# JJanai/back2future

Measured on AMD Instinct MI355X. Metric: frame-triplets/sec at 3x1024x1920, higher is better.
Workload: dtype f32; 1 GPU; BASELINE.json configs[4] per-GPU share: batch=16 synthetic 3x1024x1920 triplets per GPU, random-init pwc.lua weights (Ours-Hard shape), outputs flow + occ + est[3]; batch_per_gpu=16, global_batch=16, height=1024, width=1920, parallelism=dp1: independent triplets per rank, one RCCL weight broadcast at init, hip_graph=True

## Files before the change

back2future_amd/csrc/b2f_api.hip:

```cpp
#include "b2f_ctx.h"

#include <cctype>
#include <cmath>
#include <cstdio>
#include <cstdlib>

using namespace b2f;

static thread_local std::string g_err;
namespace b2f {
int api_fail(const std::string &m)
{
    g_err = m;
    return 1;
}
const std::string &api_error() { return g_err; }

ConvSeg cp8_seg(const float *ptr, int C, size_t hw)
{
    ConvSeg sgm;
    sgm.ptr = ptr;
    sgm.img_stride = (long)(hw * (size_t)((C + 7) / 8 * 8));
    sgm.chunk_stride = (long)(hw * 8);
    sgm.pix_stride = 8;
// ... 240 lines not shown
    return 0;
}

int find_conv(const b2f_ctx *c, int kind, int level, int idx)
{
    for (size_t i = 0; i < c->lay.size(); ++i)
        if (c->lay[i].kind == kind && c->lay[i].level == level && c->lay[i].idx == idx) return (int)i;
    return -1;
}

struct Plan {
    int B, H, W;
    bool full;
    bool seq;
    bool stream;
    bool past;
    int nimg;
    int fo;
    int rec;
    int h[8], w[8];
    size_t img, tmp, cs[8], U[8], UB[8], cv, d[6], fs, bfs, logits, u2, flow_planar, ds[6], total;
};

Plan make_plan(int B, int H, int W, bool full, bool past_flow, bool seq = false, bool stream = false, bool want_past = false)
{
    Plan p;
    p.B = B; p.H = H; p.W = W;
    p.full = full;
    p.seq = seq;
    p.stream = stream;
    p.past = past_flow && (full || want_past);
    p.nimg = stream ? B : seq ? B + 2 : 3 * B;
    p.fo = seq ? 1 : B;
    p.rec = kCvRec;
    for (int l = 1; l <= 7; ++l) { p.h[l] = H >> (l - 1); p.w[l] = W >> (l - 1); }
    size_t off = 0;
    auto take = [&](size_t n) { size_t o = off; off += (n + 63) & ~(size_t)63; return o; };
    p.img = full ? take((size_t)3 * B * H * W * kImgC) : 0;
    p.tmp = take((size_t)p.nimg * p.h[2] * p.w[2] * kFeat[2]);
    for (int l = 2; l <= 7; ++l) p.cs[l] = take((stream && l >= 3) ? 0 : (size_t)p.nimg * p.h[l] * p.w[l] * kFeat[l]);
    for (int l = 3; l <= 6; ++l) p.U[l] = take((size_t)B * p.h[l] * p.w[l] * 2);
    for (int l = 3; l <= 6; ++l) p.UB[l] = p.past ? take((size_t)B * p.h[l] * p.w[l] * 2) : 0;
    p.cv = take((size_t)B * p.h[3] * p.w[3] * p.rec + 64);
    const size_t px3 = (size_t)B * p.h[3] * p.w[3];
    for (int i = 1; i <= 5; ++i) p.d[i] = take(px3 * kDec[i]);
    p.fs = take(px3 * 8);
    p.bfs = take(px3 * 8);
    p.logits = take(px3 * 8);
    p.u2 = take(px3 * 4 * 2);
    p.flow_planar = take((size_t)B * 2 * H * W);
    for (int k = 2; k <= 5; ++k) p.ds[k] = full ? take((size_t)2 * B * (H >> (k - 1)) * (W >> (k - 1)) * kImgC) : 0;
    p.total = off;
    return p;
}

}
void b2f::drop_gen_out(b2f_ctx *c)
{
    for (float *p : c->gen_out)
        if (p) (void)hipFree(p);
    c->gen_out.clear();
    c->genB = c->genH = c->genW = 0;
}
void b2f::drop_graphs(b2f_ctx *c)
// ... 120 lines not shown
{
    const PackedConv &p = c->packed[conv_id];
    ConvLaunch L{};
    for (int i = 0; i < p.nseg; ++i) L.seg[i] = segs[i];
    L.out = out;
    L.H = H; L.W = W; L.stride = stride;
    const size_t hwo = (size_t)((H + 2 - 3) / stride + 1) * ((W + 2 - 3) / stride + 1);
    L.out_img_stride = (long)(hwo * ((p.cout + 7) / 8 * 8));
    L.out_chunk_stride = (long)(hwo * 8);
    L.out_pix_stride = 8;
    L.nimg = nimg;
    L.leaky = leaky;
    return launch_layer(c, s, !cap, p, c->wpk_dev, *c, c->cur_batch, L);
}

int run_decoder(b2f_ctx *c, hipStream_t s, bool cap, const Plan &P, const float *ref, int kind, int l, float *out2)
{
    const size_t *dbuf = P.d;
    float *A = c->arena;
    const int h = P.h[l], w = P.w[l], B = P.B;
    const size_t hw = (size_t)h * w;
    const int Cl = kFeat[l];
    const int id1 = find_conv(c, kind, l, 1);
    if (id1 < 0) return fail("decoder not present in this model");
    ConvSeg segs[2];
    const ConvSeg seg_ref = cp8_seg(ref, Cl, hw);
    const ConvSeg seg_cv = cp8_seg(A + P.cv, kCvRec, hw);
    if (c->packed[id1].nseg == 2) { segs[0] = seg_ref; segs[1] = seg_cv; }
    else { segs[0] = seg_cv; segs[1] = seg_cv; }
    CHK(run_conv(c, s, cap, id1, segs, B, h, w, 1, 1, A + dbuf[1]));
    for (int i = 2; i <= 6; ++i) {
        const ConvSeg in = cp8_seg(A + dbuf[i - 1], kDec[i - 1], hw);
        float *o = (i == 6) ? out2 : A + dbuf[i];
        CHK(run_conv(c, s, cap, find_conv(c, kind, l, i), &in, B, h, w, 1, i < 6, o));
    }
    return 0;
}

struct Feat {
    float *pyr[8];
    const float *past[8], *ref[8], *fut[8];
};

Feat make_feat(const b2f_ctx *c, const Plan &P, const StreamPass *sp)
{
    Feat F{};
    for (int l = 2; l <= 7; ++l) {
        const size_t img = (size_t)P.h[l] * P.w[l] * kFeat[l];
        if (sp && l >= 3) {
            F.pyr[l] = sp->pyr[l];
            F.past[l] = sp->past[l]; F.ref[l] = sp->ref[l]; F.fut[l] = sp->fut[l];
// ... 7 lines not shown

struct Outs {
    float *flow = nullptr, *occ = nullptr, *est3 = nullptr;
    float *past = nullptr;
    float *t_ufs[8] = {nullptr}, *t_ubfs[8] = {nullptr}, *t_occ[8] = {nullptr}, *t_iw1[8] = {nullptr}, *t_iw3[8] = {nullptr};
};

int forward_impl(b2f_ctx *c, hipStream_t s, bool cap, const void *dev_in, int in_kind, const Plan &P, const Outs &O, const StreamPass *sp = nullptr)
{
    c->cur_batch = c->req_batch > 0 ? c->req_batch : P.B;
    float *A = c->arena;
    const Feat F = make_feat(c, P, sp);
    const int B = P.B;
    const bool full = P.full, past = P.past;
    const int unit = in_kind == B2F_IN_UNIT;
    if (full) {
        Scope sc(c, s, "pack_input", cap);
        HIPCHK(launch_pack_input((const float *)dev_in, unit, B, P.H, P.W, A + P.img, s));
    }
    const int head_id1 = find_conv(c, KIND_FEAT, 2, 2), head_id2 = find_conv(c, KIND_FEAT, 3, 1);
    const bool head_fused = c->bf16_direct >= 2 && P.h[2] >= 4 && P.w[2] >= 4 && head_id1 >= 0 && head_id2 >= 0 &&
                            c->packed[(size_t)head_id1].base == K_C16 && c->packed[(size_t)head_id2].base == K_C16S2;
    for (int l = 2; l <= 7; ++l) {
        const int hi = P.h[l - 1], wi = P.w[l - 1], ho = P.h[l], wo = P.w[l];
        const int Ci = (l == 2) ? kImgC : kFeat[l - 1], Co = kFeat[l];
        if (l == 2 && (P.seq || sp)) {
            Scope sc(c, s, "conv_first_seq", cap);
            HIPCHK(launch_conv_first_seq(dev_in, in_kind, P.nimg, P.H, P.W, c->wpk_dev + c->first_w_off, c->wpk_dev + c->first_b_off,
                                         A + P.tmp, s));
        } else if (l == 2) {
// ... 56 lines not shown
        cl.out = A + P.cv;
        cl.out_img_stride = (long)(hw * kCvRec);
        cl.out_chunk_stride = (long)(hw * 8);
        cl.out_pix_stride = 8;
        cl.B = B; cl.C = Cl; cl.h = h; cl.w = w;
        cl.variant = c->corr_variant;
        cl.ablate = c->corr_ablate;
        {
            char cname[48];
            snprintf(cname, sizeof cname, c->profile_layers ? "warp_costvol_%dx%d" : "warp_costvol", h, w);
            Scope sc(c, s, cname, cap);
            HIPCHK(launch_warp_costvol(cl, s));
        }
        float *occ_out = full ? O.t_occ[l] : (l == 3 ? O.occ : nullptr);
        float *occ_out2 = (!full && l == 3 && c->past_flow) ? O.est3 : nullptr;
        if (occ_out || occ_out2) {
            CHK(run_decoder(c, s, cap, P, F.ref[l], KIND_OCC, l, A + P.logits));
            {
                Scope sc(c, s, "softmax_nearest4", cap);
                if (occ_out) HIPCHK(launch_softmax_nearest4_planar(A + P.logits, 8, B, h, w, occ_out, s));
                if (occ_out2) HIPCHK(launch_softmax_nearest4_planar(A + P.logits, 8, B, h, w, occ_out2, s));
            }
        }
        CHK(run_decoder(c, s, cap, P, F.ref[l], KIND_FLOW, l, A + P.fs));
        if (past) CHK(run_decoder(c, s, cap, P, F.ref[l], KIND_PAST, l, A + P.bfs));
        float *skip_f = full ? O.t_ufs[l] : (l == 3 ? (O.flow ? O.flow : A + P.flow_planar) : nullptr);
        {
            Scope sc(c, s, "upsample_flow2x", cap);
            float *u = (l > 3) ? A + P.U[l - 1] : A + P.u2;
            HIPCHK(launch_upsample_flow2x(A + P.fs, 8, B, h, w, u, s));
            if (skip_f) HIPCHK(launch_upsample_flow2x_planar(u, 2, B, 2 * h, 2 * w, skip_f, s));
            if (past) {
                float *ub = (l > 3) ? A + P.UB[l - 1] : A + P.d[1];
                HIPCHK(launch_upsample_flow2x(A + P.bfs, 8, B, h, w, ub, s));
                float *skip_b = full ? O.t_ubfs[l] : (l == 3 ? O.past : nullptr);
                if (skip_b) HIPCHK(launch_upsample_flow2x_planar(ub, 2, B, 2 * h, 2 * w, skip_b, s));
            }
// ... 3 lines not shown
            const int k = l - 2;
            const int hk = 4 * h, wk = 4 * w;
            const size_t img_f = (size_t)B * hk * wk * kImgC;
            const float *im1 = (k == 1) ? A + P.img : A + P.ds[k];
            const float *im3 = (k == 1) ? A + P.img + 2 * img_f : A + P.ds[k] + img_f;
            const float kk = (float)(20.0 / std::pow(2.0, l - 3));
            const float *fl1 = (past && O.t_ubfs[l]) ? O.t_ubfs[l] : O.t_ufs[l];
            if (O.t_iw1[l]) HIPCHK(launch_warp_image_planar(im1, fl1, -kk, B, hk, wk, O.t_iw1[l], s));
            if (O.t_iw3[l]) HIPCHK(launch_warp_image_planar(im3, O.t_ufs[l], kk, B, hk, wk, O.t_iw3[l], s));
        }
    }
    if (!full && O.est3 && !c->past_flow && (P.seq || sp)) {
        Scope sc(c, s, "warp_image_seq", cap);
        HIPCHK(launch_warp_input_seq(sp ? sp->frame_past : dev_in, sp ? sp->frame_kind : in_kind, O.flow ? O.flow : A + P.flow_planar, -20.0f, B,
                                     P.H, P.W, O.est3, s));
    } else if (!full && O.est3 && !c->past_flow) {
        Scope sc(c, s, "warp_image", cap);
        HIPCHK(launch_warp_input_planar((const float *)dev_in, unit, 0, O.flow ? O.flow : A + P.flow_planar, -20.0f, B, P.H, P.W,
                                        O.est3, s));
    }
    return 0;
}

}
int b2f::find_conv_id(const b2f_ctx *c, int kind, int level, int idx) { return find_conv(c, kind, level, idx); }
int b2f::run_conv_layer(b2f_ctx *c, hipStream_t s, bool cap, int conv_id, const ConvSeg *segs, int nimg, int H, int W, int stride,
                        int leaky, float *out)
{
    if (conv_id < 0) return fail("b2f: layer not present in this model");
    return run_conv(c, s, cap, conv_id, segs, nimg, H, W, stride, leaky, out);
}
// ... 76 lines not shown
    {"bf16_conv_min_pixels", &b2f_ctx::bf16_conv_min_pixels, OPT_SYNC, 0},
    {"wino1d", &b2f_ctx::wino1d, OPT_ENV | OPT_SYNC, 2},
    {"wino6", &b2f_ctx::wino6, OPT_ENV | OPT_SYNC, 3},
    {"wino6_min_pixels", &b2f_ctx::wino6_min_pixels, OPT_ENV | OPT_SYNC, 0},
    {"wino2_split", &b2f_ctx::wino2_split, OPT_ENV | OPT_SYNC | OPT_EXP_ONLY, 4},
    {"wino4_split", &b2f_ctx::wino4_split, OPT_ENV | OPT_SYNC | OPT_EXP_ONLY, 5},
    {"wino4_hybrid", &b2f_ctx::wino4_hybrid, OPT_ENV | OPT_SYNC | OPT_EXP_ONLY, 5},
    {"s2_tiles_per_block", &b2f_ctx::s2_tiles_per_block, OPT_ENV | OPT_SYNC, 0},
    {"wino4_persistent", &b2f_ctx::wino4_persistent, OPT_ENV | OPT_SYNC, 0},
    {"s2_loader", &b2f_ctx::s2_loader, OPT_ENV | OPT_SYNC, 0},
    {"s2_tile_groups", &b2f_ctx::s2_tile_groups, OPT_ENV | OPT_SYNC, 0},
    {"wino_split_pixels", &b2f_ctx::wino_split_pixels, OPT_ENV | OPT_SYNC, 0},
    {"wino8", &b2f_ctx::wino8, OPT_ENV | OPT_SYNC, 0},
    {"wino4_min_pixels", &b2f_ctx::wino4_min_pixels, OPT_ENV | OPT_SYNC, 0},
    {"adaptive_kernels", &b2f_ctx::adaptive_kernels, OPT_ENV | OPT_SYNC, 0},
    {"op_wino_split", &b2f_ctx::op_wino_split, OPT_ENV, 0},
    {"op_hole_fill", &b2f_ctx::op_hole_fill, 0, 0},
    {"host_subbatch_pixels", nullptr, OPT_ENV, 0},
    {"host_threads", &b2f_ctx::host_threads, OPT_ENV, 0},
    {"host_u8", &b2f_ctx::host_u8, OPT_ENV, 0},
    {"host_ramp", &b2f_ctx::host_ramp, OPT_ENV, 0},
    {"debug_fail_next", &b2f_ctx::debug_fail_next, 0, 0},
};

const OptRow *find_option(const char *key)
{
    for (const OptRow &r : kOptions)
        if (!strcmp(key, r.name)) return &r;
    return nullptr;
}
// ... 350 lines not shown
                    drop_gen_out(c);
                    return fail("b2f_forward_device: out of device memory");
                }
            }
            c->genB = B; c->genH = H; c->genW = W;
        }
        std::vector<float *> &dev = c->gen_out;
        CHK(graph_forward(c, s, false, dev_in, in_kind, B, H, W, dev.data()));
        const size_t n2 = (size_t)B * 2 * H * W * sizeof(float);
        if (dev_flow) HIPCHK(hipMemcpyAsync(dev_flow, dev[0], n2, hipMemcpyDeviceToDevice, s));
        if (dev_occ) HIPCHK(hipMemcpyAsync(dev_occ, dev[(size_t)(c->past_flow ? 2 : 1)], n2, hipMemcpyDeviceToDevice, s));
        if (dev_est3) HIPCHK(hipMemcpyAsync(dev_est3, dev[2], c->past_flow ? n2 : n2 / 2 * 3, hipMemcpyDeviceToDevice, s));
        if (dev_past) HIPCHK(hipMemcpyAsync(dev_past, dev[1], n2, hipMemcpyDeviceToDevice, s));
        return 0;
    }
    const Plan P = make_plan(B, H, W, false, c->past_flow, seq, sp != nullptr, dev_past != nullptr);
    CHK(ensure_workspace(c, P));
    Outs O;
    O.flow = dev_flow; O.occ = dev_occ; O.est3 = dev_est3; O.past = dev_past;
    if (graph && !c->profile) {
        if (c->graphs.size() > 256) {
            HIPCHK(hipDeviceSynchronize());
            drop_graphs(c);
        }
        const int req = c->req_batch > 0 ? c->req_batch : B;
        const GraphKey key = {dev_in, dev_flow, dev_occ, dev_est3, in_kind, B, H, W, (c->adaptive_kernels > 0 || (c->adaptive_kernels < 0 && req == 1)) ? 1 : 0,
                              seq ? 1 : 0, sp ? sp->ring : nullptr, sp ? 1 + 2 * sp->slot + (sp->ready ? 1 : 0) : 0, dev_past};
        auto it = c->graphs.find(key);
        if (it == c->graphs.end()) {
            c->graphs.emplace(key, nullptr);
            return forward_impl(c, s, false, dev_in, in_kind, P, O, sp);
// ... 664 lines not shown
```

back2future_amd/csrc/b2f_ctx.h:

```cpp
#pragma once
#include "../../include/b2f.h"

#include <algorithm>
#include <atomic>
#include <condition_variable>
#include <cstring>
#include <exception>
#include <map>
#include <memory>
#include <mutex>
#include <string>
#include <thread>
#include <tuple>
#include <vector>

#include "b2f_host.h"
#include "b2f_internal.h"

namespace b2f {

int api_fail(const std::string &m);
const std::string &api_error();


// ... 357 lines not shown
    float *wpk_dev = nullptr;
    size_t wpk_floats = 0;
    size_t first_w_off = 0, first_b_off = 0;
    float *arena = nullptr;
    size_t arena_floats = 0;
    int wsB = 0, wsH = 0, wsW = 0;
    int use_graph = 0, profile = 0;
    int host_graph = 1;
    int cur_batch = 0;
    int req_batch = 0;
    int corr_ablate = 0;
    int corr_variant = -1;
    int op_wino_split = 0;
    int op_hole_fill = 0;
    int profile_layers = 0;
    long long host_subbatch_pixels = 16ll << 20;
    int host_threads = 0;
    int host_u8 = 1, host_ramp = 1;
    int debug_fail_next = 0;
    std::map<b2f::GraphKey, hipGraphExec_t> graphs;
    std::vector<float *> gen_out;
    int genB = 0, genH = 0, genW = 0;
    std::vector<std::string> prof_names;
    std::vector<double> prof_ms;
    std::vector<long long> prof_n;
    std::vector<b2f::ProfEvent> prof_pending;
    std::vector<hipEvent_t> ev_pool;
    hipStream_t s_in = nullptr, s_out = nullptr;
    b2f::HostSlot slot[2];
    std::unique_ptr<b2f::CopyPool> pool_in, pool_out;
// ... 46 lines not shown
```

back2future_amd/csrc/b2f_glue.hip:

```cpp
#include "b2f_internal.h"

namespace b2f {

__global__ void pack_input_kernel(const float *in, int normalize, int B, int H, int W, float *img)
{
    const size_t hw = (size_t)H * W;
    const size_t i = (size_t)blockIdx.x * blockDim.x + threadIdx.x;
    if (i >= (size_t)B * hw) return;
    const size_t b = i / hw, p = i - b * hw;
#pragma unroll
    for (int f = 0; f < 3; ++f) {
        float v[3];
#pragma unroll
        for (int c = 0; c < 3; ++c) {
            float x = in[(b * 9 + f * 3 + c) * hw + p];
            if (normalize) x = color_normalize(x, c);
            v[c] = x;
        }
        float4 *o = reinterpret_cast<float4 *>(img + (((size_t)f * B + b) * hw + p) * kImgC);
        o[0] = make_float4(v[0], v[1], v[2], 0.f);
        o[1] = make_float4(0.f, 0.f, 0.f, 0.f);
    }
}

// ... 30 lines not shown
    const float bl = y1 ? src[(size_t)iw * pix_stride] : 0.f;
    const float br = (x1 && y1) ? src[(size_t)(iw + 1) * pix_stride] : 0.f;
    out[pix * out_pix_stride + c] = wx * wy * tl + (1.f - wx) * wy * tr + wx * (1.f - wy) * bl + (1.f - wx) * (1.f - wy) * br;
}

hipError_t launch_warp_nhwc(const float *img, long img_stride, int pix_stride, int C, int ih, int iw,
                            const float *grid, float k, int B, int gh, int gw, float *out,
                            int out_pix_stride, hipStream_t s)
{
    const size_t n = (size_t)B * gh * gw * C;
    hipLaunchKernelGGL(warp_nhwc_kernel, dim3((unsigned)((n + 255) / 256)), dim3(256), 0, s, img, img_stride,
                       pix_stride, C, ih, iw, grid, k, B, gh, gw, out, out_pix_stride);
    return hipGetLastError();
}

__device__ __forceinline__ float2 bilerp2(const float *in, int ps, int h, int w, float rh, float rw, int y2, int x2)
{
    const float h1r = rh * (float)y2;
    const int h1 = (int)h1r;
    const int h1p = (h1 < h - 1) ? 1 : 0;
    const float h1l = h1r - (float)h1, h0l = 1.f - h1l;
    const float w1r = rw * (float)x2;
    const int w1 = (int)w1r;
    const int w1p = (w1 < w - 1) ? 1 : 0;
    const float w1l = w1r - (float)w1, w0l = 1.f - w1l;
    const float *p = in + ((size_t)h1 * w + w1) * ps;
    const float2 a = *reinterpret_cast<const float2 *>(p), b = *reinterpret_cast<const float2 *>(p + (size_t)w1p * ps);
    const float2 c = *reinterpret_cast<const float2 *>(p + (size_t)h1p * w * ps);
    const float2 d = *reinterpret_cast<const float2 *>(p + ((size_t)h1p * w + w1p) * ps);
    float2 o;
    o.x = h0l * (w0l * a.x + w1l * b.x) + h1l * (w0l * c.x + w1l * d.x);
    o.y = h0l * (w0l * a.y + w1l * b.y) + h1l * (w0l * c.y + w1l * d.y);
    return o;
}

__global__ __launch_bounds__(256) void upsample_flow2x_kernel(const float *in, int ps, int B, int h, int w, float *out, int planar)
{
    const int H2 = 2 * h, W2 = 2 * w;
    const int x0 = 4 * (int)(blockIdx.x * blockDim.x + threadIdx.x);
    const int y2 = (int)blockIdx.y, b = (int)blockIdx.z;
    if (x0 >= W2) return;
    const float rh = (H2 > 1) ? (float)(h - 1) / (float)(H2 - 1) : 0.f;
    const float rw = (W2 > 1) ? (float)(w - 1) / (float)(W2 - 1) : 0.f;
    const float *src = in + (size_t)b * h * w * ps;
    float2 o[4];
#pragma unroll
    for (int k = 0; k < 4; ++k) o[k] = bilerp2(src, ps, h, w, rh, rw, y2, min(x0 + k, W2 - 1));
    const size_t hw2 = (size_t)H2 * W2, row = (size_t)y2 * W2 + x0;
    if (planar) {
        float *o0 = out + ((size_t)b * 2) * hw2 + row, *o1 = o0 + hw2;
        if ((W2 & 3) == 0) {
            *reinterpret_cast<float4 *>(o0) = make_float4(o[0].x, o[1].x, o[2].x, o[3].x);
            *reinterpret_cast<float4 *>(o1) = make_float4(o[0].y, o[1].y, o[2].y, o[3].y);
        } else {
#pragma unroll
            for (int k = 0; k < 4; ++k)
                if (x0 + k < W2) { o0[k] = o[k].x; o1[k] = o[k].y; }
        }
// ... 16 lines not shown
    if (2 * h > 65535 || B > 65535) return hipErrorInvalidValue;
    const int groups = (2 * w + 3) / 4;
    hipLaunchKernelGGL(upsample_flow2x_kernel, dim3((unsigned)((groups + 255) / 256), (unsigned)(2 * h), (unsigned)B), dim3(256), 0, s, in,
                       in_pix_stride, B, h, w, out, planar);
    return hipGetLastError();
}
hipError_t launch_upsample_flow2x(const float *in, int in_pix_stride, int B, int h, int w, float *out, hipStream_t s)
{
    return launch_upsample(in, in_pix_stride, B, h, w, out, 0, s);
}
hipError_t launch_upsample_flow2x_planar(const float *in, int in_pix_stride, int B, int h, int w, float *out, hipStream_t s)
{
    return launch_upsample(in, in_pix_stride, B, h, w, out, 1, s);
}

__global__ __launch_bounds__(256) void softmax_nearest4_kernel(const float *logits, int ps, int B, int h, int w, float *out)
{
    const int H4 = 4 * h, W4 = 4 * w;
    const int x = (int)(blockIdx.x * blockDim.x + threadIdx.x);
    const int Y = (int)blockIdx.y, b = (int)blockIdx.z;
    if (x >= w) return;
    const float2 z = *reinterpret_cast<const float2 *>(logits + (((size_t)b * h + (Y >> 2)) * w + x) * ps);
    const float m = fmaxf(z.x, z.y);
    const float e0 = expf(z.x - m), e1 = expf(z.y - m);
    const float sum = e0 + e1;
    const float p0 = e0 / sum, p1 = e1 / sum;
    const size_t hw4 = (size_t)H4 * W4;
    float *o0 = out + ((size_t)b * 2) * hw4 + (size_t)Y * W4 + 4 * x;
    *reinterpret_cast<float4 *>(o0) = make_float4(p0, p0, p0, p0);
    *reinterpret_cast<float4 *>(o0 + hw4) = make_float4(p1, p1, p1, p1);
}

hipError_t launch_softmax_nearest4_planar(const float *logits, int in_pix_stride, int B, int h, int w, float *out, hipStream_t s)
{
    if (B <= 0 || h <= 0 || w <= 0) return hipSuccess;
    if (4 * h > 65535 || B > 65535) return hipErrorInvalidValue;
    hipLaunchKernelGGL(softmax_nearest4_kernel, dim3((unsigned)((w + 255) / 256), (unsigned)(4 * h), (unsigned)B), dim3(256), 0, s, logits,
                       in_pix_stride, B, h, w, out);
    return hipGetLastError();
}

// ... 114 lines not shown
    *reinterpret_cast<float4 *>(op + 4) = make_float4(acc[4], acc[5], acc[6], acc[7]);
    *reinterpret_cast<float4 *>(op + hwo * 8) = make_float4(acc[8], acc[9], acc[10], acc[11]);
    *reinterpret_cast<float4 *>(op + hwo * 8 + 4) = make_float4(acc[12], acc[13], acc[14], acc[15]);
}

hipError_t launch_conv_first(const float *in, int normalize, int B, int H, int W, const float *wt, const float *bias,
                             float *out, hipStream_t s)
{
    const int Ho = H / 2, Wo = W / 2;
    const int tiles = ((Wo + 31) / 32) * ((Ho + 7) / 8);
    hipLaunchKernelGGL(conv_first_kernel, dim3((unsigned)(tiles * 3 * B)), dim3(256), 0, s, in, normalize, B, H, W, wt, bias, out);
    return hipGetLastError();
}

template <int CPB>
__global__ __launch_bounds__(256) void conv_narrow2_kernel(const float *in, long img_stride, long chunk_stride, int pix_stride,
                                                           int nchunks, int H, int W, const float *wt, const float *bias,
                                                           float *out, long out_img_stride, int out_pix_stride, int leaky)
{
    constexpr int T = 16, P = T + 2, NP = P * P;
    __shared__ float4 patch[CPB][2][NP + 4];
    __shared__ float4 wsh[CPB * 36];
    const int tiles_x = (W + T - 1) / T, tiles_y = (H + T - 1) / T;
    int bid = blockIdx.x;
    const int tx_i = bid % tiles_x;
    bid /= tiles_x;
    const int ty_i = bid % tiles_y;
    const int img = bid / tiles_y;
    const int ox0 = tx_i * T, oy0 = ty_i * T;
    const int ty = threadIdx.x >> 4, tx = threadIdx.x & 15;
    const float *src = in + (size_t)img * img_stride;
    float a0 = bias[0], a1 = bias[1];
    for (int c0 = 0; c0 < nchunks; c0 += CPB) {
        const int nc = min(CPB, nchunks - c0);
        if (c0) __syncthreads();
        constexpr int NIT = (CPB * 2 * NP + 255) / 256;
        float4 v[NIT];
        bool ok[NIT];
#pragma unroll
        for (int k = 0; k < NIT; ++k) {
            const int i = threadIdx.x + k * 256;
            const int c = i / (2 * NP), r = i - c * (2 * NP);
            const int pix = r >> 1, k4 = r & 1;
            const int py = pix / P, px = pix - py * P;
            const int gy = oy0 - 1 + py, gx = ox0 - 1 + px;
            ok[k] = i < nc * 2 * NP && gy >= 0 && gy < H && gx >= 0 && gx < W;
            v[k] = *reinterpret_cast<const float4 *>(src + (size_t)(ok[k] ? c0 + c : 0) * chunk_stride +
// ... 17 lines not shown
                    const int pp = (ty + ky) * P + tx + kx;
                    const float4 lo = patch[c][0][pp], hi = patch[c][1][pp];
                    const float4 *wk = wsh + (c * 9 + ky * 3 + kx) * 4;
                    const float4 w0 = wk[0], w1 = wk[1], w2 = wk[2], w3 = wk[3];
                    a0 = fmaf(lo.x, w0.x, a0);  a1 = fmaf(lo.x, w0.y, a1);
                    a0 = fmaf(lo.y, w0.z, a0);  a1 = fmaf(lo.y, w0.w, a1);
                    a0 = fmaf(lo.z, w1.x, a0);  a1 = fmaf(lo.z, w1.y, a1);
                    a0 = fmaf(lo.w, w1.z, a0);  a1 = fmaf(lo.w, w1.w, a1);
                    a0 = fmaf(hi.x, w2.x, a0);  a1 = fmaf(hi.x, w2.y, a1);
                    a0 = fmaf(hi.y, w2.z, a0);  a1 = fmaf(hi.y, w2.w, a1);
                    a0 = fmaf(hi.z, w3.x, a0);  a1 = fmaf(hi.z, w3.y, a1);
                    a0 = fmaf(hi.w, w3.z, a0);  a1 = fmaf(hi.w, w3.w, a1);
                }
        }
    }
    const int oy = oy0 + ty, ox = ox0 + tx;
    if (oy >= H || ox >= W) return;
    if (leaky) { a0 = a0 > 0.f ? a0 : 0.2f * a0; a1 = a1 > 0.f ? a1 : 0.2f * a1; }
    float *op = out + (size_t)img * out_img_stride + ((size_t)oy * W + ox) * out_pix_stride;
    *reinterpret_cast<float2 *>(op) = make_float2(a0, a1);
}

hipError_t launch_conv_narrow2(const ConvLaunch &p, hipStream_t s)
{
    if (p.stride != 1 || p.cout != 2 || p.nseg != 1 || (p.seg[0].pix_stride & 3) || (p.out_pix_stride & 1)) return hipErrorInvalidValue;
    const int tiles = ((p.W + 15) / 16) * ((p.H + 15) / 16);
    if ((long)tiles * p.nimg <= 3L * device_cu_count() && p.seg[0].nchunks > 2)
        hipLaunchKernelGGL(conv_narrow2_kernel<4>, dim3((unsigned)(tiles * p.nimg)), dim3(256), 0, s, p.seg[0].ptr, p.seg[0].img_stride,
                           p.seg[0].chunk_stride, p.seg[0].pix_stride, p.seg[0].nchunks, p.H, p.W, p.wpk, p.bias, p.out,
                           p.out_img_stride, p.out_pix_stride, p.leaky);
// ... 8 lines not shown

void narrow2_pack_weights(const float *w, const float *b, int Ci, const int *cin_map, int cin_chunks, float *wpk, float *bpk)
{
    for (int c = 0; c < cin_chunks; ++c)
        for (int t = 0; t < 9; ++t)
            for (int j = 0; j < 8; ++j)
                for (int o = 0; o < 2; ++o) {
                    const int k = c * kCK + j;
                    const int ci = cin_map ? cin_map[k] : (k < Ci ? k : -1);
                    wpk[((c * 9 + t) * 8 + j) * 2 + o] = ci >= 0 ? w[((size_t)o * Ci + ci) * 9 + t] : 0.f;
                }
    bpk[0] = b[0];
    bpk[1] = b[1];
}

__global__ void warp_input_planar_kernel(const float *in, int normalize, int frame, const float *flow, float k, int B,
                                         int H, int W, float *out)
{
    const size_t hw = (size_t)H * W;
    const size_t i = (size_t)blockIdx.x * blockDim.x + threadIdx.x;
    if (i >= (size_t)B * hw) return;
    const size_t b = i / hw, p = i - b * hw;
    const int y = (int)(p / W), x = (int)(p - (size_t)y * W);
    const float u = flow[(b * 2) * hw + p] * k, v = flow[(b * 2 + 1) * hw + p] * k;
    int xl, yt;
    float wx, wy;
    bhwd_top_left(u + (float)x, W, xl, wx);
    bhwd_top_left(v + (float)y, H, yt, wy);
    const int dx = (xl + 1 <= W - 1) ? 1 : 0, dy = (yt + 1 <= H - 1) ? W : 0;
    const float w00 = wx * wy, w01 = (1.f - wx) * wy, w10 = wx * (1.f - wy), w11 = (1.f - wx) * (1.f - wy);
#pragma unroll
    for (int c = 0; c < 3; ++c) {
        const float *src = in + (b * 9 + (size_t)frame * 3 + c) * hw + (size_t)yt * W + xl;
        float tl = src[0], tr = src[dx], bl = src[dy], br = src[dy + dx];
        if (normalize) {
            tl = color_normalize(tl, c); tr = color_normalize(tr, c);
            bl = color_normalize(bl, c); br = color_normalize(br, c);
        }
        out[(b * 3 + c) * hw + p] = w00 * tl + w01 * tr + w10 * bl + w11 * br;
    }
}

hipError_t launch_warp_input_planar(const float *in, int normalize, int frame, const float *flow_planar, float k, int B,
                                    int H, int W, float *out, hipStream_t s)
{
    const size_t n = (size_t)B * H * W;
    hipLaunchKernelGGL(warp_input_planar_kernel, dim3((unsigned)((n + 255) / 256)), dim3(256), 0, s, in, normalize, frame,
                       flow_planar, k, B, H, W, out);
    return hipGetLastError();
}

__global__ void avgpool2_kernel(const float *in, int nimg, int H, int W, int C, float *out)
{
    const int Ho = H / 2, Wo = W / 2, C4 = C / 4;
    const size_t n = (size_t)nimg * Ho * Wo * C4;
    const size_t i = (size_t)blockIdx.x * blockDim.x + threadIdx.x;
    if (i >= n) return;
    const int c4 = (int)(i % C4);
    size_t pix = i / C4;
    const int X = (int)(pix % Wo);
    const size_t r = pix / Wo;
    const int Y = (int)(r % Ho);
    const size_t b = r / Ho;
    const float4 *s = reinterpret_cast<const float4 *>(in) + ((b * H + 2 * Y) * W + 2 * X) * C4 + c4;
    const float4 a = s[0], bb = s[C4], c = s[(size_t)W * C4], d = s[(size_t)(W + 1) * C4];
// ... 90 lines not shown
```

back2future_amd/csrc/b2f_internal.h:

```cpp
#pragma once
#include <hip/hip_runtime.h>
#ifndef B2F_EXPERIMENTS
#define B2F_EXPERIMENTS 0
#endif
#include <cstdint>

namespace b2f {

constexpr int kLevels = 7, kLst = 3, kWin = 9, kND = 2 * kWin * kWin;
constexpr int kFeat[8] = {0, 3, 16, 32, 64, 96, 128, 192};
constexpr int kDec[7] = {0, 128, 128, 96, 64, 32, 2};
constexpr int kCvRec = 168;
constexpr int kCvChunks = 21;
constexpr int kImgC = 8;
constexpr int kCK = 8;

struct ConvSeg {
    const float *ptr;
    long img_stride;
    long chunk_stride;
    int pix_stride;
    int nchunks;
};
struct ConvLaunch {
// ... 71 lines not shown
    float *out;
    long out_img_stride, out_chunk_stride;
    int out_pix_stride;
    int Ho, Wo, nimg;
    int rows_per_block, nsy, nsx;
    long long *trace = nullptr;
};
bool head16_supported(const HeadLaunch &p);
hipError_t launch_conv_head16(HeadLaunch p, hipStream_t s);
bool c16s2_supported(const ConvLaunch &p);
hipError_t launch_conv3x3_c16s2(const ConvLaunch &p, hipStream_t s);
size_t c16s2_wpk_floats();
void c16s2_pack_weights(const float *w, const float *b, int Ci, const int *cin_map, float *wpk, float *bpk);
hipError_t launch_conv_narrow2(const ConvLaunch &p, hipStream_t s);
size_t narrow2_wpk_floats(int cin_chunks);
void narrow2_pack_weights(const float *w, const float *b, int Ci, const int *cin_map, int cin_chunks, float *wpk, float *bpk);
hipError_t launch_conv3x3_wino(const ConvLaunch &p, hipStream_t s);
void wino_choose_tiles(int cout, int *nt, int *nblk);
size_t wino_wpk_floats(int cin_chunks, int nt, int nblk);
hipError_t launch_conv3x3_wino4(const ConvLaunch &p, hipStream_t s);
hipError_t launch_conv3x3_wino4_rem(const ConvLaunch &p, hipStream_t s);
bool wino4s_supported(const ConvLaunch &p);
hipError_t launch_conv3x3_wino4s(const ConvLaunch &p, int nb0, int nblk, hipStream_t s);
size_t wino4s_wpk_floats(int cin_chunks, int nblk);
bool wino2s_supported(const ConvLaunch &p);
hipError_t launch_conv3x3_wino2s(const ConvLaunch &p, int nb0, int nblk, hipStream_t s);
size_t wino2s_wpk_floats(int cin_chunks, int nblk);
void wino2s_pack_weights(const float *w, int Co, int Ci, const int *cin_map, int cin_chunks, int nblk, float *wpk);
void wino4s_pack_weights(const float *w, int Co, int Ci, const int *cin_map, int cin_chunks, int nblk, float *wpk);
int wino4_nblk(int cout);
// ... 140 lines not shown
```

Measured before the change: 865.8 triplets/s.

## Fuse narrow2 decoder heads with upsample, softmax and image warp epilogues

Adds fused kernels in which the final 2-channel narrow2 conv of each decoder computes its tile and then, inside the same block, performs the bilinear 2x flow upsample, the softmax plus nearest-4 occupancy expansion, or the double upsample to full resolution followed by the image warp. This removes the intermediate fs/bfs/logits/u2 buffers along with the extra kernel launches and global round trips they required. In exchange the kernels recompute halo pixels in shared memory, tiles are smaller, and the conv tile work is duplicated across overlapping halos. The path is enabled by default through fused_heads=1, which fuses only the l>3 and occ heads; level 3 plus the warp needs fused_heads=2.

```diff
diff --git a/back2future_amd/csrc/b2f_api.hip b/back2future_amd/csrc/b2f_api.hip
--- a/back2future_amd/csrc/b2f_api.hip
+++ b/back2future_amd/csrc/b2f_api.hip
@@ -278,6 +278,7 @@
     bool full;
     bool seq;
     bool stream;
+    int fused;
     bool past;
     int nimg;
     int fo;
@@ -286,7 +287,7 @@
     size_t img, tmp, cs[8], U[8], UB[8], cv, d[6], fs, bfs, logits, u2, flow_planar, ds[6], total;
 };
 
-Plan make_plan(int B, int H, int W, bool full, bool past_flow, bool seq = false, bool stream = false, bool want_past = false)
+Plan make_plan(int B, int H, int W, bool full, bool past_flow, bool seq = false, bool stream = false, bool want_past = false, int fused = 0)
 {
     Plan p;
     p.B = B; p.H = H; p.W = W;
@@ -294,6 +295,7 @@
     p.seq = seq;
     p.stream = stream;
     p.past = past_flow && (full || want_past);
+    p.fused = full ? 0 : fused;
     p.nimg = stream ? B : seq ? B + 2 : 3 * B;
     p.fo = seq ? 1 : B;
     p.rec = kCvRec;
@@ -308,10 +310,11 @@
     p.cv = take((size_t)B * p.h[3] * p.w[3] * p.rec + 64);
     const size_t px3 = (size_t)B * p.h[3] * p.w[3];
     for (int i = 1; i <= 5; ++i) p.d[i] = take(px3 * kDec[i]);
-    p.fs = take(px3 * 8);
-    p.bfs = take(px3 * 8);
-    p.logits = take(px3 * 8);
-    p.u2 = take(px3 * 4 * 2);
+    const size_t px3f = p.fused >= 2 ? 0 : px3;
+    p.fs = take(px3f * 8);
+    p.bfs = take(px3f * 8);
+    p.logits = take(p.fused ? 0 : px3 * 8);
+    p.u2 = take(px3f * 4 * 2);
     p.flow_planar = take((size_t)B * 2 * H * W);
     for (int k = 2; k <= 5; ++k) p.ds[k] = full ? take((size_t)2 * B * (H >> (k - 1)) * (W >> (k - 1)) * kImgC) : 0;
     p.total = off;
@@ -462,7 +465,7 @@
     return launch_layer(c, s, !cap, p, c->wpk_dev, *c, c->cur_batch, L);
 }
 
-int run_decoder(b2f_ctx *c, hipStream_t s, bool cap, const Plan &P, const float *ref, int kind, int l, float *out2)
+int run_decoder(b2f_ctx *c, hipStream_t s, bool cap, const Plan &P, const float *ref, int kind, int l, float *out2, Narrow2Head *head = nullptr)
 {
     const size_t *dbuf = P.d;
     float *A = c->arena;
@@ -479,10 +482,34 @@
     CHK(run_conv(c, s, cap, id1, segs, B, h, w, 1, 1, A + dbuf[1]));
     for (int i = 2; i <= 6; ++i) {
         const ConvSeg in = cp8_seg(A + dbuf[i - 1], kDec[i - 1], hw);
+        if (i == 6 && head) {
+            const int id6 = find_conv(c, kind, l, 6);
+            if (id6 < 0 || c->packed[(size_t)id6].base != K_NARROW2 || c->packed[(size_t)id6].nseg != 1) return fail("fused_heads: the decoder's last layer has no narrow2 packing");
+            const PackedConv &p6 = c->packed[(size_t)id6];
+            head->in = in;
+            head->in.nchunks = p6.chunks[0];
+            head->H = h; head->W = w; head->nimg = B; head->leaky = 0;
+            head->wpk = c->wpk_dev + p6.pk[K_NARROW2].w_off;
+            head->bias = c->wpk_dev + p6.pk[K_NARROW2].b_off;
+            break;
+        }
         float *o = (i == 6) ? out2 : A + dbuf[i];
         CHK(run_conv(c, s, cap, find_conv(c, kind, l, i), &in, B, h, w, 1, i < 6, o));
     }
     return 0;
+}
+
+int heads_fused(const b2f_ctx *c)
+{
+    const int id = find_conv(c, KIND_FLOW, 3, 6);
+    return (id >= 0 && c->packed[(size_t)id].base == K_NARROW2) ? std::max(0, std::min(c->fused_heads, 2)) : 0;
+}
+
+const char *head_row(const b2f_ctx *c, const Narrow2Head &hd, const char *cls, char (&name)[48])
+{
+    if (!c->profile_layers) return cls;
+    snprintf(name, sizeof name, "conv%s_%dto2_%dx%d", kKernels[K_NARROW2].tag[0], hd.in.nchunks * 8, hd.H, hd.W);
+    return name;
 }
 
 struct Feat {
@@ -520,6 +547,7 @@
     const int B = P.B;
     const bool full = P.full, past = P.past;
     const int unit = in_kind == B2F_IN_UNIT;
+    const bool warp_fused = P.fused >= 2 && O.est3 && !c->past_flow && !(P.seq || sp);
     if (full) {
         Scope sc(c, s, "pack_input", cap);
         HIPCHK(launch_pack_input((const float *)dev_in, unit, B, P.H, P.W, A + P.img, s));
@@ -606,13 +634,38 @@
         }
         float *occ_out = full ? O.t_occ[l] : (l == 3 ? O.occ : nullptr);
         float *occ_out2 = (!full && l == 3 && c->past_flow) ? O.est3 : nullptr;
-        if (occ_out || occ_out2) {
+        char hname[48];
+        if ((occ_out || occ_out2) && P.fused) {
+            Narrow2Head hd;
+            CHK(run_decoder(c, s, cap, P, F.ref[l], KIND_OCC, l, nullptr, &hd));
+            Scope sc(c, s, head_row(c, hd, "conv3x3_narrow2", hname), cap);
+            HIPCHK(launch_occ_head(hd, occ_out, occ_out2, s));
+        } else if (occ_out || occ_out2) {
             CHK(run_decoder(c, s, cap, P, F.ref[l], KIND_OCC, l, A + P.logits));
             {
                 Scope sc(c, s, "softmax_nearest4", cap);
                 if (occ_out) HIPCHK(launch_softmax_nearest4_planar(A + P.logits, 8, B, h, w, occ_out, s));
                 if (occ_out2) HIPCHK(launch_softmax_nearest4_planar(A + P.logits, 8, B, h, w, occ_out2, s));
             }
+        }
+        if (P.fused >= (l > 3 ? 1 : 2)) {
+            for (int dir = 0; dir < (past ? 2 : 1); ++dir) {
+                if (l == 3 && dir && !O.past) continue;
+                Narrow2Head hd;
+                CHK(run_decoder(c, s, cap, P, F.ref[l], dir ? KIND_PAST : KIND_FLOW, l, nullptr, &hd));
+                if (l > 3) {
+                    Scope sc(c, s, head_row(c, hd, "conv3x3_narrow2", hname), cap);
+                    HIPCHK(launch_narrow2_up(hd, A + (dir ? P.UB[l - 1] : P.U[l - 1]), s));
+                } else if (dir) {
+                    Scope sc(c, s, head_row(c, hd, "conv3x3_narrow2", hname), cap);
+                    HIPCHK(launch_flow_tail(hd, O.past, nullptr, 0, 0.f, nullptr, s));
+                } else {
+                    float *dst = O.flow ? O.flow : (warp_fused ? nullptr : A + P.flow_planar);
+                    Scope sc(c, s, head_row(c, hd, warp_fused ? "warp_image" : "conv3x3_narrow2", hname), cap);
+                    HIPCHK(launch_flow_tail(hd, dst, warp_fused ? (const float *)dev_in : nullptr, unit, -20.0f, warp_fused ? O.est3 : nullptr, s));
+                }
+            }
+            continue;
         }
         CHK(run_decoder(c, s, cap, P, F.ref[l], KIND_FLOW, l, A + P.fs));
         if (past) CHK(run_decoder(c, s, cap, P, F.ref[l], KIND_PAST, l, A + P.bfs));
@@ -646,7 +699,7 @@
         Scope sc(c, s, "warp_image_seq", cap);
         HIPCHK(launch_warp_input_seq(sp ? sp->frame_past : dev_in, sp ? sp->frame_kind : in_kind, O.flow ? O.flow : A + P.flow_planar, -20.0f, B,
                                      P.H, P.W, O.est3, s));
-    } else if (!full && O.est3 && !c->past_flow) {
+    } else if (!full && O.est3 && !c->past_flow && !warp_fused) {
         Scope sc(c, s, "warp_image", cap);
         HIPCHK(launch_warp_input_planar((const float *)dev_in, unit, 0, O.flow ? O.flow : A + P.flow_planar, -20.0f, B, P.H, P.W,
                                         O.est3, s));
@@ -753,6 +806,7 @@
     {"wino8", &b2f_ctx::wino8, OPT_ENV | OPT_SYNC, 0},
     {"wino4_min_pixels", &b2f_ctx::wino4_min_pixels, OPT_ENV | OPT_SYNC, 0},
     {"adaptive_kernels", &b2f_ctx::adaptive_kernels, OPT_ENV | OPT_SYNC, 0},
+    {"fused_heads", &b2f_ctx::fused_heads, OPT_ENV | OPT_SYNC, 0},
     {"op_wino_split", &b2f_ctx::op_wino_split, OPT_ENV, 0},
     {"op_hole_fill", &b2f_ctx::op_hole_fill, 0, 0},
     {"host_subbatch_pixels", nullptr, OPT_ENV, 0},
@@ -1133,7 +1187,7 @@
         if (dev_past) HIPCHK(hipMemcpyAsync(dev_past, dev[1], n2, hipMemcpyDeviceToDevice, s));
         return 0;
     }
-    const Plan P = make_plan(B, H, W, false, c->past_flow, seq, sp != nullptr, dev_past != nullptr);
+    const Plan P = make_plan(B, H, W, false, c->past_flow, seq, sp != nullptr, dev_past != nullptr, heads_fused(c));
     CHK(ensure_workspace(c, P));
     Outs O;
     O.flow = dev_flow; O.occ = dev_occ; O.est3 = dev_est3; O.past = dev_past;
diff --git a/back2future_amd/csrc/b2f_ctx.h b/back2future_amd/csrc/b2f_ctx.h
--- a/back2future_amd/csrc/b2f_ctx.h
+++ b/back2future_amd/csrc/b2f_ctx.h
@@ -395,6 +395,7 @@
     int op_wino_split = 0;
     int op_hole_fill = 0;
     int profile_layers = 0;
+    int fused_heads = 1;
     long long host_subbatch_pixels = 16ll << 20;
     int host_threads = 0;
     int host_u8 = 1, host_ramp = 1;
diff --git a/back2future_amd/csrc/b2f_glue.hip b/back2future_amd/csrc/b2f_glue.hip
--- a/back2future_amd/csrc/b2f_glue.hip
+++ b/back2future_amd/csrc/b2f_glue.hip
@@ -68,25 +68,47 @@
     return hipGetLastError();
 }
 
+struct Lerp2 {
+    int i1, ip;
+    float l1, l0;
+};
+__device__ __forceinline__ Lerp2 bilerp_axis(float r, int n, int o2)
+{
+    Lerp2 a;
+    const float h1r = r * (float)o2;
+    a.i1 = (int)h1r;
+    a.ip = (a.i1 < n - 1) ? 1 : 0;
+    a.l1 = h1r - (float)a.i1;
+    a.l0 = 1.f - a.l1;
+    return a;
+}
+__device__ __forceinline__ float2 bilerp_blend(float2 a, float2 b, float2 c, float2 d, const Lerp2 &y, const Lerp2 &x)
+{
+    const float h0l = y.l0, h1l = y.l1, w0l = x.l0, w1l = x.l1;
+    float2 o;
+    o.x = h0l * (w0l * a.x + w1l * b.x) + h1l * (w0l * c.x + w1l * d.x);
+    o.y = h0l * (w0l * a.y + w1l * b.y) + h1l * (w0l * c.y + w1l * d.y);
+    return o;
+}
 __device__ __forceinline__ float2 bilerp2(const float *in, int ps, int h, int w, float rh, float rw, int y2, int x2)
 {
-    const float h1r = rh * (float)y2;
-    const int h1 = (int)h1r;
-    const int h1p = (h1 < h - 1) ? 1 : 0;
-    const float h1l = h1r - (float)h1, h0l = 1.f - h1l;
-    const float w1r = rw * (float)x2;
-    const int w1 = (int)w1r;
-    const int w1p = (w1 < w - 1) ? 1 : 0;
-    const float w1l = w1r - (float)w1, w0l = 1.f - w1l;
+    const Lerp2 y = bilerp_axis(rh, h, y2), x = bilerp_axis(rw, w, x2);
+    const int h1 = y.i1, h1p = y.ip, w1 = x.i1, w1p = x.ip;
     const float *p = in + ((size_t)h1 * w + w1) * ps;
     const float2 a = *reinterpret_cast<const float2 *>(p), b = *reinterpret_cast<const float2 *>(p + (size_t)w1p * ps);
     const float2 c = *reinterpret_cast<const float2 *>(p + (size_t)h1p * w * ps);
     const float2 d = *reinterpret_cast<const float2 *>(p + ((size_t)h1p * w + w1p) * ps);
-    float2 o;
-    o.x = h0l * (w0l * a.x + w1l * b.x) + h1l * (w0l * c.x + w1l * d.x);
-    o.y = h0l * (w0l * a.y + w1l * b.y) + h1l * (w0l * c.y + w1l * d.y);
-    return o;
-}
+    return bilerp_blend(a, b, c, d, y, x);
+}
+template <int T>
+__device__ __forceinline__ float2 bilerp2_tile(const float2 *tile, int ty0, int tx0, int h, int w, float rh, float rw, int y2, int x2)
+{
+    const Lerp2 y = bilerp_axis(rh, h, y2), x = bilerp_axis(rw, w, x2);
+    const int r0 = min(max(y.i1 - ty0, 0), T - 1), r1 = min(max(y.i1 + y.ip - ty0, 0), T - 1);
+    const int c0 = min(max(x.i1 - tx0, 0), T - 1), c1 = min(max(x.i1 + x.ip - tx0, 0), T - 1);
+    return bilerp_blend(tile[r0 * T + c0], tile[r0 * T + c1], tile[r1 * T + c0], tile[r1 * T + c1], y, x);
+}
+__host__ __device__ __forceinline__ float up2_ratio(int n) { return (2 * n > 1) ? (float)(n - 1) / (float)(2 * n - 1) : 0.f; }
 
 __global__ __launch_bounds__(256) void upsample_flow2x_kernel(const float *in, int ps, int B, int h, int w, float *out, int planar)
 {
@@ -94,8 +116,7 @@
     const int x0 = 4 * (int)(blockIdx.x * blockDim.x + threadIdx.x);
     const int y2 = (int)blockIdx.y, b = (int)blockIdx.z;
     if (x0 >= W2) return;
-    const float rh = (H2 > 1) ? (float)(h - 1) / (float)(H2 - 1) : 0.f;
-    const float rw = (W2 > 1) ? (float)(w - 1) / (float)(W2 - 1) : 0.f;
+    const float rh = up2_ratio(h), rw = up2_ratio(w);
     const float *src = in + (size_t)b * h * w * ps;
     float2 o[4];
 #pragma unroll
@@ -142,17 +163,22 @@
     return launch_upsample(in, in_pix_stride, B, h, w, out, 1, s);
 }
 
+__device__ __forceinline__ float2 softmax2(float2 z)
+{
+    const float m = fmaxf(z.x, z.y);
+    const float e0 = expf(z.x - m), e1 = expf(z.y - m);
+    const float sum = e0 + e1;
+    return make_float2(e0 / sum, e1 / sum);
+}
+
 __global__ __launch_bounds__(256) void softmax_nearest4_kernel(const float *logits, int ps, int B, int h, int w, float *out)
 {
     const int H4 = 4 * h, W4 = 4 * w;
     const int x = (int)(blockIdx.x * blockDim.x + threadIdx.x);
     const int Y = (int)blockIdx.y, b = (int)blockIdx.z;
     if (x >= w) return;
-    const float2 z = *reinterpret_cast<const float2 *>(logits + (((size_t)b * h + (Y >> 2)) * w + x) * ps);
-    const float m = fmaxf(z.x, z.y);
-    const float e0 = expf(z.x - m), e1 = expf(z.y - m);
-    const float sum = e0 + e1;
-    const float p0 = e0 / sum, p1 = e1 / sum;
+    const float2 p = softmax2(*reinterpret_cast<const float2 *>(logits + (((size_t)b * h + (Y >> 2)) * w + x) * ps));
+    const float p0 = p.x, p1 = p.y;
     const size_t hw4 = (size_t)H4 * W4;
     float *o0 = out + ((size_t)b * 2) * hw4 + (size_t)Y * W4 + 4 * x;
     *reinterpret_cast<float4 *>(o0) = make_float4(p0, p0, p0, p0);
@@ -297,23 +323,14 @@
 }
 
 template <int CPB>
-__global__ __launch_bounds__(256) void conv_narrow2_kernel(const float *in, long img_stride, long chunk_stride, int pix_stride,
-                                                           int nchunks, int H, int W, const float *wt, const float *bias,
-                                                           float *out, long out_img_stride, int out_pix_stride, int leaky)
+__device__ __forceinline__ void narrow2_tile(const float *src, long chunk_stride, int pix_stride, int nchunks, int H, int W, int oy0, int ox0,
+                                             const float *wt, const float *bias, float &a0, float &a1)
 {
     constexpr int T = 16, P = T + 2, NP = P * P;
     __shared__ float4 patch[CPB][2][NP + 4];
     __shared__ float4 wsh[CPB * 36];
-    const int tiles_x = (W + T - 1) / T, tiles_y = (H + T - 1) / T;
-    int bid = blockIdx.x;
-    const int tx_i = bid % tiles_x;
-    bid /= tiles_x;
-    const int ty_i = bid % tiles_y;
-    const int img = bid / tiles_y;
-    const int ox0 = tx_i * T, oy0 = ty_i * T;
     const int ty = threadIdx.x >> 4, tx = threadIdx.x & 15;
-    const float *src = in + (size_t)img * img_stride;
-    float a0 = bias[0], a1 = bias[1];
+    a0 = bias[0]; a1 = bias[1];
     for (int c0 = 0; c0 < nchunks; c0 += CPB) {
         const int nc = min(CPB, nchunks - c0);
         if (c0) __syncthreads();
@@ -361,6 +378,24 @@
                 }
         }
     }
+}
+
+template <int CPB>
+__global__ __launch_bounds__(256) void conv_narrow2_kernel(const float *in, long img_stride, long chunk_stride, int pix_stride,
+                                                           int nchunks, int H, int W, const float *wt, const float *bias,
+                                                           float *out, long out_img_stride, int out_pix_stride, int leaky)
+{
+    constexpr int T = 16;
+    const int tiles_x = (W + T - 1) / T, tiles_y = (H + T - 1) / T;
+    int bid = blockIdx.x;
+    const int tx_i = bid % tiles_x;
+    bid /= tiles_x;
+    const int ty_i = bid % tiles_y;
+    const int img = bid / tiles_y;
+    const int ox0 = tx_i * T, oy0 = ty_i * T;
+    const int ty = threadIdx.x >> 4, tx = threadIdx.x & 15;
+    float a0, a1;
+    narrow2_tile<CPB>(in + (size_t)img * img_stride, chunk_stride, pix_stride, nchunks, H, W, oy0, ox0, wt, bias, a0, a1);
     const int oy = oy0 + ty, ox = ox0 + tx;
     if (oy >= H || ox >= W) return;
     if (leaky) { a0 = a0 > 0.f ? a0 : 0.2f * a0; a1 = a1 > 0.f ? a1 : 0.2f * a1; }
@@ -399,15 +434,11 @@
     bpk[1] = b[1];
 }
 
-__global__ void warp_input_planar_kernel(const float *in, int normalize, int frame, const float *flow, float k, int B,
-                                         int H, int W, float *out)
+__device__ __forceinline__ void warp_input_pixel(const float *in, int normalize, int frame, float fu, float fv, float k, size_t b, int y, int x,
+                                                 int H, int W, float o[3])
 {
     const size_t hw = (size_t)H * W;
-    const size_t i = (size_t)blockIdx.x * blockDim.x + threadIdx.x;
-    if (i >= (size_t)B * hw) return;
-    const size_t b = i / hw, p = i - b * hw;
-    const int y = (int)(p / W), x = (int)(p - (size_t)y * W);
-    const float u = flow[(b * 2) * hw + p] * k, v = flow[(b * 2 + 1) * hw + p] * k;
+    const float u = fu * k, v = fv * k;
     int xl, yt;
     float wx, wy;
     bhwd_top_left(u + (float)x, W, xl, wx);
@@ -422,8 +453,22 @@
             tl = color_normalize(tl, c); tr = color_normalize(tr, c);
             bl = color_normalize(bl, c); br = color_normalize(br, c);
         }
-        out[(b * 3 + c) * hw + p] = w00 * tl + w01 * tr + w10 * bl + w11 * br;
-    }
+        o[c] = w00 * tl + w01 * tr + w10 * bl + w11 * br;
+    }
+}
+
+__global__ void warp_input_planar_kernel(const float *in, int normalize, int frame, const float *flow, float k, int B,
+                                         int H, int W, float *out)
+{
+    const size_t hw = (size_t)H * W;
+    const size_t i = (size_t)blockIdx.x * blockDim.x + threadIdx.x;
+    if (i >= (size_t)B * hw) return;
+    const size_t b = i / hw, p = i - b * hw;
+    const int y = (int)(p / W), x = (int)(p - (size_t)y * W);
+    float o[3];
+    warp_input_pixel(in, normalize, frame, flow[(b * 2) * hw + p], flow[(b * 2 + 1) * hw + p], k, b, y, x, H, W, o);
+#pragma unroll
+    for (int c = 0; c < 3; ++c) out[(b * 3 + c) * hw + p] = o[c];
 }
 
 hipError_t launch_warp_input_planar(const float *in, int normalize, int frame, const float *flow_planar, float k, int B,
@@ -434,6 +479,197 @@
                        flow_planar, k, B, H, W, out);
     return hipGetLastError();
 }
+
+constexpr int kHeadOwn = 14;
+
+static bool up2_reads_within(int n, int tiles, int out_first, int out_step, int out_count, int src_first, int src_step, int src_count)
+{
+    const float r = up2_ratio(n);
+    for (int t = 0; t < tiles; ++t) {
+        const int o0 = out_first + t * out_step, s0 = src_first + t * src_step;
+        for (int o = o0 > 0 ? o0 : 0; o < o0 + out_count && o < 2 * n; ++o) {
+            const int i1 = (int)(r * (float)o), ip = (i1 < n - 1) ? 1 : 0;
+            if (i1 < s0 || i1 + ip >= s0 + src_count) return false;
+        }
+    }
+    return true;
+}
+static bool up_halo_ok(int n)
+{
+    return up2_reads_within(n, (n + kHeadOwn - 1) / kHeadOwn, 0, 2 * kHeadOwn, 2 * kHeadOwn, -1, kHeadOwn, 16);
+}
+static bool tail_halo_ok(int n)
+{
+    const int tiles = (n + kHeadOwn - 1) / kHeadOwn;
+    return up2_reads_within(2 * n, tiles, 0, 4 * kHeadOwn, 4 * kHeadOwn, -1, 2 * kHeadOwn, 2 * kHeadOwn + 2) &&
+           up2_reads_within(n, tiles, -1, 2 * kHeadOwn, 2 * kHeadOwn + 2, -1, kHeadOwn, 16);
+}
+
+struct HeadTile {
+    int tx_i, ty_i, img;
+};
+__device__ __forceinline__ HeadTile head_tile(int H, int W, int own)
+{
+    const int tiles_x = (W + own - 1) / own, tiles_y = (H + own - 1) / own;
+    HeadTile t;
+    int bid = blockIdx.x;
+    t.tx_i = bid % tiles_x;
+    bid /= tiles_x;
+    t.ty_i = bid % tiles_y;
+    t.img = bid / tiles_y;
+    return t;
+}
+
+template <int CPB>
+__global__ __launch_bounds__(256) void narrow2_up_kernel(const float *in, long img_stride, long chunk_stride, int pix_stride, int nchunks,
+                                                         int H, int W, const float *wt, const float *bias, int leaky, float *out)
+{
+    __shared__ float2 fs[16 * 16];
+    const HeadTile t = head_tile(H, W, kHeadOwn);
+    const int oy0 = t.ty_i * kHeadOwn - 1, ox0 = t.tx_i * kHeadOwn - 1;
+    float a0, a1;
+    narrow2_tile<CPB>(in + (size_t)t.img * img_stride, chunk_stride, pix_stride, nchunks, H, W, oy0, ox0, wt, bias, a0, a1);
+    if (leaky) { a0 = a0 > 0.f ? a0 : 0.2f * a0; a1 = a1 > 0.f ? a1 : 0.2f * a1; }
+    fs[threadIdx.x] = make_float2(a0, a1);
+    __syncthreads();
+    const int H2 = 2 * H, W2 = 2 * W;
+    const float rh = up2_ratio(H), rw = up2_ratio(W);
+    float2 *dst = reinterpret_cast<float2 *>(out) + (size_t)t.img * H2 * W2;
+    for (int i = threadIdx.x; i < 2 * kHeadOwn * kHeadOwn; i += 256) {
+        const int ry = i / kHeadOwn, rx = i - ry * kHeadOwn;
+        const int y2 = t.ty_i * 2 * kHeadOwn + ry, x2 = t.tx_i * 2 * kHeadOwn + 2 * rx;
+        if (y2 >= H2 || x2 >= W2) continue;
+        const float2 o0 = bilerp2_tile<16>(fs, oy0, ox0, H, W, rh, rw, y2, x2), o1 = bilerp2_tile<16>(fs, oy0, ox0, H, W, rh, rw, y2, x2 + 1);
+        *reinterpret_cast<float4 *>(dst + (size_t)y2 * W2 + x2) = make_float4(o0.x, o0.y, o1.x, o1.y);
+    }
+}
+
+template <int CPB, bool WARP>
+__global__ __launch_bounds__(256) void flow_tail_kernel(const float *in, long img_stride, long chunk_stride, int pix_stride, int nchunks,
+                                                        int H, int W, const float *wt, const float *bias, int leaky, float *flow,
+                                                        const float *frames, int normalize, float k, float *est3)
+{
+    constexpr int U = 2 * kHeadOwn + 2;
+    __shared__ float2 fs[16 * 16];
+    __shared__ float2 u2[U * U];
+    const HeadTile t = head_tile(H, W, kHeadOwn);
+    const int oy0 = t.ty_i * kHeadOwn - 1, ox0 = t.tx_i * kHeadOwn - 1;
+    float a0, a1;
+    narrow2_tile<CPB>(in + (size_t)t.img * img_stride, chunk_stride, pix_stride, nchunks, H, W, oy0, ox0, wt, bias, a0, a1);
+    if (leaky) { a0 = a0 > 0.f ? a0 : 0.2f * a0; a1 = a1 > 0.f ? a1 : 0.2f * a1; }
+    fs[threadIdx.x] = make_float2(a0, a1);
+    __syncthreads();
+    const int H2 = 2 * H, W2 = 2 * W, H4 = 4 * H, W4 = 4 * W;
+    const int uy0 = t.ty_i * 2 * kHeadOwn - 1, ux0 = t.tx_i * 2 * kHeadOwn - 1;
+    {
+        const float rh = up2_ratio(H), rw = up2_ratio(W);
+        for (int i = threadIdx.x; i < U * U; i += 256) {
+            const int ry = i / U, rx = i - ry * U;
+            const int y2 = uy0 + ry, x2 = ux0 + rx;
+            if (y2 >= 0 && y2 < H2 && x2 >= 0 && x2 < W2) u2[i] = bilerp2_tile<16>(fs, oy0, ox0, H, W, rh, rw, y2, x2);
+        }
+    }
+    __syncthreads();
+    const float rh = up2_ratio(H2), rw = up2_ratio(W2);
+    const size_t hw4 = (size_t)H4 * W4;
+    for (int i = threadIdx.x; i < 4 * kHeadOwn * kHeadOwn; i += 256) {
+        const int ry = i / kHeadOwn, rx = i - ry * kHeadOwn;
+        const int y4 = t.ty_i * 4 * kHeadOwn + ry, x4 = t.tx_i * 4 * kHeadOwn + 4 * rx;
+        if (y4 >= H4 || x4 >= W4) continue;
+        float2 o[4];
+#pragma unroll
+        for (int j = 0; j < 4; ++j) o[j] = bilerp2_tile<U>(u2, uy0, ux0, H2, W2, rh, rw, y4, x4 + j);
+        const size_t row = (size_t)y4 * W4 + x4;
+        if (flow) {
+            float *o0 = flow + ((size_t)t.img * 2) * hw4 + row;
+            *reinterpret_cast<float4 *>(o0) = make_float4(o[0].x, o[1].x, o[2].x, o[3].x);
+            *reinterpret_cast<float4 *>(o0 + hw4) = make_float4(o[0].y, o[1].y, o[2].y, o[3].y);
+        }
+        if (WARP) {
+            float e[4][3];
+#pragma unroll
+            for (int j = 0; j < 4; ++j) warp_input_pixel(frames, normalize, 0, o[j].x, o[j].y, k, (size_t)t.img, y4, x4 + j, H4, W4, e[j]);
+#pragma unroll
+            for (int c = 0; c < 3; ++c)
+                *reinterpret_cast<float4 *>(est3 + ((size_t)t.img * 3 + c) * hw4 + row) = make_float4(e[0][c], e[1][c], e[2][c], e[3][c]);
+        }
+    }
+}
+
+template <int CPB>
+__global__ __launch_bounds__(256) void occ_head_kernel(const float *in, long img_stride, long chunk_stride, int pix_stride, int nchunks,
+                                                       int H, int W, const float *wt, const float *bias, int leaky, float *occ, float *occ2)
+{
+    const HeadTile t = head_tile(H, W, 16);
+    const int oy0 = t.ty_i * 16, ox0 = t.tx_i * 16;
+    float a0, a1;
+    narrow2_tile<CPB>(in + (size_t)t.img * img_stride, chunk_stride, pix_stride, nchunks, H, W, oy0, ox0, wt, bias, a0, a1);
+    const int oy = oy0 + (int)(threadIdx.x >> 4), ox = ox0 + (int)(threadIdx.x & 15);
+    if (oy >= H || ox >= W) return;
+    if (leaky) { a0 = a0 > 0.f ? a0 : 0.2f * a0; a1 = a1 > 0.f ? a1 : 0.2f * a1; }
+    const float2 p = softmax2(make_float2(a0, a1));
+    const int W4 = 4 * W;
+    const size_t hw4 = (size_t)4 * H * W4;
+    const size_t at = ((size_t)t.img * 2) * hw4 + (size_t)(4 * oy) * W4 + 4 * ox;
+    const float4 p0 = make_float4(p.x, p.x, p.x, p.x), p1 = make_float4(p.y, p.y, p.y, p.y);
+#pragma unroll
+    for (int r = 0; r < 4; ++r) {
+        if (occ) {
+            *reinterpret_cast<float4 *>(occ + at + (size_t)r * W4) = p0;
+            *reinterpret_cast<float4 *>(occ + at + hw4 + (size_t)r * W4) = p1;
+        }
+        if (occ2) {
+            *reinterpret_cast<float4 *>(occ2 + at + (size_t)r * W4) = p0;
+            *reinterpret_cast<float4 *>(occ2 + at + hw4 + (size_t)r * W4) = p1;
+        }
+    }
+}
+
+static bool head_one_pass(const Narrow2Head &p, long blocks) { return blocks <= 3L * device_cu_count() && p.in.nchunks > 2; }
+static bool head_args_ok(const Narrow2Head &p)
+{
+    return p.H > 0 && p.W > 0 && p.nimg > 0 && !(p.in.pix_stride & 3) && p.in.nchunks > 0;
+}
+#define HEAD_ARGS p.in.ptr, p.in.img_stride, p.in.chunk_stride, p.in.pix_stride, p.in.nchunks, p.H, p.W, p.wpk, p.bias, p.leaky
+
+hipError_t launch_narrow2_up(const Narrow2Head &p, float *out, hipStream_t s)
+{
+    if (!head_args_ok(p) || !out) return hipErrorInvalidValue;
+    const int ty = (p.H + kHeadOwn - 1) / kHeadOwn, tx = (p.W + kHeadOwn - 1) / kHeadOwn;
+    if (!up_halo_ok(p.H) || !up_halo_ok(p.W)) return hipErrorAssert;
+    const long blocks = (long)ty * tx * p.nimg;
+    if (head_one_pass(p, blocks))
+        hipLaunchKernelGGL(narrow2_up_kernel<4>, dim3((unsigned)blocks), dim3(256), 0, s, HEAD_ARGS, out);
+    else
+        hipLaunchKernelGGL(narrow2_up_kernel<2>, dim3((unsigned)blocks), dim3(256), 0, s, HEAD_ARGS, out);
+    return hipGetLastError();
+}
+
+hipError_t launch_flow_tail(const Narrow2Head &p, float *flow, const float *frames, int normalize, float k, float *est3, hipStream_t s)
+{
+    if (!head_args_ok(p) || (!flow && !est3) || (est3 && !frames)) return hipErrorInvalidValue;
+    const int ty = (p.H + kHeadOwn - 1) / kHeadOwn, tx = (p.W + kHeadOwn - 1) / kHeadOwn;
+    if (!tail_halo_ok(p.H) || !tail_halo_ok(p.W)) return hipErrorAssert;
+    const long blocks = (long)ty * tx * p.nimg;
+    const bool one = head_one_pass(p, blocks);
+#define TAIL(CPB, WARP) hipLaunchKernelGGL((flow_tail_kernel<CPB, WARP>), dim3((unsigned)blocks), dim3(256), 0, s, HEAD_ARGS, flow, frames, normalize, k, est3)
+    if (est3) { if (one) TAIL(4, true); else TAIL(2, true); }
+    else { if (one) TAIL(4, false); else TAIL(2, false); }
+#undef TAIL
+    return hipGetLastError();
+}
+
+hipError_t launch_occ_head(const Narrow2Head &p, float *occ, float *occ2, hipStream_t s)
+{
+    if (!head_args_ok(p) || (!occ && !occ2)) return hipErrorInvalidValue;
+    const long blocks = (long)((p.H + 15) / 16) * ((p.W + 15) / 16) * p.nimg;
+    if (head_one_pass(p, blocks))
+        hipLaunchKernelGGL(occ_head_kernel<4>, dim3((unsigned)blocks), dim3(256), 0, s, HEAD_ARGS, occ, occ2);
+    else
+        hipLaunchKernelGGL(occ_head_kernel<2>, dim3((unsigned)blocks), dim3(256), 0, s, HEAD_ARGS, occ, occ2);
+    return hipGetLastError();
+}
+#undef HEAD_ARGS
 
 __global__ void avgpool2_kernel(const float *in, int nimg, int H, int W, int C, float *out)
 {
diff --git a/back2future_amd/csrc/b2f_internal.h b/back2future_amd/csrc/b2f_internal.h
--- a/back2future_amd/csrc/b2f_internal.h
+++ b/back2future_amd/csrc/b2f_internal.h
@@ -109,6 +109,14 @@
 void c16s2_pack_weights(const float *w, const float *b, int Ci, const int *cin_map, float *wpk, float *bpk);
 hipError_t launch_conv_narrow2(const ConvLaunch &p, hipStream_t s);
 size_t narrow2_wpk_floats(int cin_chunks);
+struct Narrow2Head {
+    ConvSeg in;
+    int H, W, nimg, leaky;
+    const float *wpk, *bias;
+};
+hipError_t launch_narrow2_up(const Narrow2Head &p, float *out, hipStream_t s);
+hipError_t launch_flow_tail(const Narrow2Head &p, float *flow, const float *frames, int normalize, float k, float *est3, hipStream_t s);
+hipError_t launch_occ_head(const Narrow2Head &p, float *occ, float *occ2, hipStream_t s);
 void narrow2_pack_weights(const float *w, const float *b, int Ci, const int *cin_map, int cin_chunks, float *wpk, float *bpk);
 hipError_t launch_conv3x3_wino(const ConvLaunch &p, hipStream_t s);
 void wino_choose_tiles(int cout, int *nt, int *nblk);
```

Result: no change. 868.6 triplets/s, median of 3 (+0.3%).
